# sunbains/scann-rust

Hardware: AMD Instinct MI355X
Metric: QPS @ recall10@10 + achieved HBM GB/s, 1M x 128 f32 (higher is better)
Workload: dtype f32; 1 GPU; AsymmetricHasher LUT16 S=32 K=16 + exact re-rank; n=1000000, n_per_gpu=1000000, dim=128, k=10, batch=1024, global_batch=1024, caller_streams=2, pre_reorder_k=5000, distribution=uniform, parallelism=single GPU

## Files before the change

include/scann_hip.h:

```cpp
#ifndef SCANN_HIP_H
#define SCANN_HIP_H

#include <stddef.h>
#include <stdint.h>

#ifdef __cplusplus
extern "C" {
#endif

typedef enum {
    SCANN_HIP_OK = 0,
    SCANN_HIP_CANCELLED = 1,
    SCANN_HIP_UNKNOWN = 2,
    SCANN_HIP_INVALID_ARGUMENT = 3,
    SCANN_HIP_DEADLINE_EXCEEDED = 4,
    SCANN_HIP_NOT_FOUND = 5,
    SCANN_HIP_ALREADY_EXISTS = 6,
    SCANN_HIP_PERMISSION_DENIED = 7,
    SCANN_HIP_RESOURCE_EXHAUSTED = 8,
    SCANN_HIP_FAILED_PRECONDITION = 9,
    SCANN_HIP_ABORTED = 10,
    SCANN_HIP_OUT_OF_RANGE = 11,
    SCANN_HIP_UNIMPLEMENTED = 12,
    SCANN_HIP_INTERNAL = 13,
// ... 63 lines not shown
    uint32_t pre_reorder_k;
    int32_t exact_reorder;
    uint32_t *tokens;
    float *token_dists;
    uint32_t *cand_idx;
    float *cand_dist;
    uint32_t *cand_count;
    const uint64_t *allow_bitmap;
    uint64_t allow_bitmap_bits;
    int32_t bf_exact;
} scann_hip_search_opts;

void scann_hip_search_opts_default(scann_hip_search_opts *opts);

int scann_hip_search_batched(scann_hip_index *index, const float *queries, uint32_t nq,
                             uint32_t q_stride, uint32_t q_dim, uint32_t k,
                             const scann_hip_search_opts *opts, uint32_t *out_idx,
                             float *out_dist, uint32_t *out_count);

int scann_hip_search_batched_params(scann_hip_index *index, const float *queries, uint32_t nq,
                                    uint32_t q_stride, uint32_t q_dim, const uint32_t *k_per_query,
                                    const scann_hip_search_opts *opts, uint32_t out_pitch,
                                    uint32_t *out_idx, float *out_dist, uint32_t *out_count);

int scann_hip_index_reserve(scann_hip_index *index, uint32_t max_nq, uint32_t max_k,
                            const scann_hip_search_opts *opts);
int scann_hip_search_batched_device(scann_hip_index *index, const float *d_queries,
                                    uint32_t nq, uint32_t q_stride, uint32_t k,
                                    const scann_hip_search_opts *opts, uint32_t *d_out_idx,
                                    float *d_out_dist, uint32_t *d_out_count,
                                    void *hip_stream);
int scann_hip_index_last_device_status(scann_hip_index *index, void *hip_stream);
int scann_hip_index_debug_filter_bounds(scann_hip_index *index, void *hip_stream, uint32_t nq, uint64_t *out_bounds);

#define SCANN_HIP_CROWD_MAX_DEPTH 8192
#define SCANN_HIP_CROWD_MAX_SLOTS 12288
uint32_t scann_hip_crowd_table_slots(uint32_t depth);
int scann_hip_index_set_crowding_attributes(scann_hip_index *index, const uint64_t *attrs, uint64_t n_attrs);
int scann_hip_search_crowded(scann_hip_index *index, const float *queries, uint32_t nq, uint32_t q_stride,
                             uint32_t q_dim, uint32_t k, uint32_t depth, uint32_t per_crowd_limit,
                             const scann_hip_search_opts *opts, uint32_t *out_idx, float *out_dist,
                             uint32_t *out_count);
int scann_hip_index_reserve_crowded(scann_hip_index *index, uint32_t max_nq, uint32_t max_k, uint32_t max_depth,
                                    const scann_hip_search_opts *opts);
int scann_hip_search_crowded_device(scann_hip_index *index, const float *d_queries, uint32_t nq, uint32_t q_stride,
                                    uint32_t k, uint32_t depth, uint32_t per_crowd_limit,
                                    const scann_hip_search_opts *opts, uint32_t *d_out_idx, float *d_out_dist,
                                    uint32_t *d_out_count, void *hip_stream);

#define SCANN_HIP_CROWD_MAX_DIMS 8
int scann_hip_index_set_crowding_attributes_md(scann_hip_index *index, const uint64_t *attrs, uint32_t n_dims,
                                               uint64_t n_attrs);
int scann_hip_search_crowded_md(scann_hip_index *index, const float *queries, uint32_t nq, uint32_t q_stride,
                                uint32_t q_dim, uint32_t k, uint32_t depth, const uint32_t *limits, uint32_t n_limits,
                                const scann_hip_search_opts *opts, uint32_t *out_idx, float *out_dist,
                                uint32_t *out_count);
int scann_hip_search_crowded_md_device(scann_hip_index *index, const float *d_queries, uint32_t nq, uint32_t q_stride,
                                       uint32_t k, uint32_t depth, const uint32_t *limits, uint32_t n_limits,
                                       const scann_hip_search_opts *opts, uint32_t *d_out_idx, float *d_out_dist,
                                       uint32_t *d_out_count, void *hip_stream);
int scann_hip_crowd_md_apply(scann_hip_index *index, const uint32_t *rows_idx, const float *rows_dist,
                             const uint32_t *rows_count, uint32_t nq, uint32_t depth, uint32_t k, const uint32_t *limits,
                             uint32_t n_limits, uint32_t *out_idx, float *out_dist, uint32_t *out_count);

#define SCANN_HIP_MMR_MAX_DEPTH 2048
int scann_hip_search_mmr(scann_hip_index *index, const float *queries, uint32_t nq, uint32_t q_stride, uint32_t q_dim,
// ... 148 lines not shown
```

scann_rust_amd/csrc/api.hip:

```cpp
#include <algorithm>
#include <cmath>
#include <cstddef>
#include <cstdio>
#include <cstdlib>
#include <atomic>
#include <chrono>
#include <cstring>
#include <memory>
#include <mutex>
#include <string>
#include <vector>

#include "bf.h"
#include "comm.h"
#include "common.h"
#include "crowd.h"
#include "index_arrays.h"
#include "mmr.h"
#include "mutable.h"
#include "knobs.h"
#include "launch.h"
#include "txh.h"

namespace scann {
// ... 990 lines not shown
    const uint64_t rtp = (uint64_t)kResThreads * kScanPPT;
    const uint64_t res_chunks_per_leaf = std::max<uint64_t>(1, (t.n_local / std::max(1u, L)) / rtp);
    const uint64_t qgroups = std::max<uint64_t>(1, (quads_per_leaf + kResQuads - 1) / kResQuads);
    const uint64_t units = (t.n_local / rtp + L) * qgroups;
    p.res_cl = (uint32_t)std::min<uint64_t>(64, std::max<uint64_t>(8, units / 4096));
    const bool res_layout = t.code_bits == 4 && t.S <= 32;
    bool resident = res_layout && res_chunks_per_leaf >= 8 && quads_per_leaf >= 32 && units / p.res_cl >= 1536;
    if (kn.resident == 0) resident = false;
    if (kn.resident == 2) resident = res_layout;
    if (kn.res_cl) p.res_cl = kn.res_cl;
    const bool mfma_ok = t.code_bits == 4 && !p.no_threshold && !t.exact_scan;
    const bool sparse = (uint64_t)m * 128 <= stream;
    TxhScan mfma = TxhScan::Gather;
    if (mfma_ok && sparse) mfma = quads_per_leaf >= 6 ? TxhScan::Mfma32 : quads_per_leaf >= 2 ? TxhScan::Mfma16 : TxhScan::Gather;
    if (kn.mfma == 0) mfma = TxhScan::Gather;
    if (kn.mfma == 2) mfma = mfma_ok ? TxhScan::Mfma32 : TxhScan::Gather;
    if (kn.mfma == 3) mfma = mfma_ok ? TxhScan::Mfma16 : TxhScan::Gather;
    if (mfma_ok && t.codes_sp && quads_per_leaf >= 2 && t.n_local / std::max(1u, L) >= 4096 && kn.smfmac &&
        kn.mfma != 0 && kn.mfma != 3)
        mfma = TxhScan::Smfmac;
    if (mfma == TxhScan::Mfma32 && t.codes_sp && kn.smfmac) mfma = TxhScan::Smfmac;
    p.scan = t.exact_scan ? TxhScan::Exact : mfma != TxhScan::Gather ? mfma : resident ? TxhScan::Resident : TxhScan::Gather;
    if (txh_scan_is_mfma(p.scan)) {
        p.cap32 = (uint32_t)std::min<uint64_t>(ms, (uint64_t)p.cap * 4 + 16384);
    }
    p.sp_words = kn.sp_words < 0 ? !t.ah_mode : kn.sp_words != 0;
    p.codes_in_list = t.ah_mode != 0;
    p.thr_ties = kn.thr_ties;
    p.thr_tail = kn.thr_tail && !p.no_threshold && sample_rank(m, p.st) <= kThrTailMaxRank && p.scap > 4096;
    p.sample_mfma = kn.sample_mfma && p.thr_tail && p.thr_ties && txh_scan_is_mfma(p.scan) && t.ah_mode && t.L == 1 &&
                    P == 1 && t.code_bits == 4;
    p.select_direct = kn.select_direct;
    p.use_i8 = t.rows8 && exact_reorder && m >= kn.rerank_i8_min && m > 4 * k;
    p.local_prune = kn.local_prune;
    *out = p;
    return SCANN_HIP_OK;
}

static const char *txh_kernel_name(const TxhIndexDev &t, const TxhPlan &p, bool pinned) {
    if (pinned) return p.pipeline == TxhPipeline::Wide ? "wide_scan_kernel" : "small_scan_kernel";
    switch (p.scan) {
        case TxhScan::Exact: return "leaf_exact_scan_kernel";
        case TxhScan::Mfma16: return "adc_mfma16_kernel";
        case TxhScan::Smfmac: return t.S > 32 ? "adc_smfmac_wide_kernel" : "adc_smfmac_kernel";
        case TxhScan::Mfma32: return "adc_mfma_kernel";
        case TxhScan::Resident: return "adc_scan_res_kernel";
        default: return "adc_scan_kernel";
    }
}

}

int scann::txh_resolve_m(scann_hip_index *ix, uint32_t k, const scann_hip_search_opts *opts, uint32_t *out_m) {
    if (!ix || ix->kind != KIND_TXH) return fail(SCANN_HIP_INVALID_ARGUMENT, "not a tree index");
    scann_hip_search_opts o;
    if (opts) o = *opts; else scann_hip_search_opts_default(&o);
    o.exact_reorder = 1;
    TxhPlan p;
    SCANN_TRY(plan_txh_search(ix, k, &o, 0, false, TxhPipeline::Staged, read_knobs(), &p));
    *out_m = p.m;
    return SCANN_HIP_OK;
}

extern "C" {

static int ensure_txh_workspace(scann_hip_index *ix, TxhWorkspace &s, const TxhPlan &p, bool own_queries,
// ... 634 lines not shown
    for (auto &d : ix->dslots)
        if (d.used && d.key == st && d.ws) {
            ws = d.ws;
            bfw = d.bfw;
        }
    if (ix->kind == KIND_BF) return bf_last_status(*bfw, st);
    if (ix->kind != KIND_TXH || !ws->counters.p) return SCANN_HIP_OK;
    uint32_t counters[CNT_N];
    SCANN_HIP_CHECK(hipMemcpyAsync(counters, ws->counters.p, sizeof(counters),
                                   hipMemcpyDeviceToHost, st));
    SCANN_HIP_CHECK(hipStreamSynchronize(st));
    if (counters[CNT_STATUS] != SCANN_HIP_OK)
        return fail((int)counters[CNT_STATUS],
                    "candidate threshold/buffer miss on the device path (use the host entry "
                    "point, which retries without a threshold and with a full-size buffer)");
    return SCANN_HIP_OK;
}

int scann_hip_index_debug_filter_bounds(scann_hip_index *ix, void *hip_stream, uint32_t nq, uint64_t *out_bounds) {
    if (!ix || ix->kind != KIND_TXH) return fail(SCANN_HIP_INVALID_ARGUMENT, "not a tree / hasher index");
    if (nq && !out_bounds) return fail(SCANN_HIP_INVALID_ARGUMENT, "out_bounds is null");
    SCANN_TRY(set_device(ix->ctx));
    hipStream_t st = static_cast<hipStream_t>(hip_stream);
    std::lock_guard<std::mutex> lock(ix->mu);
    const TxhWorkspace *ws = &ix->ws;
    for (auto &d : ix->dslots)
        if (d.used && d.key == st && d.ws) ws = d.ws;
    if (!ws->thr.p || ws->thr.bytes < (size_t)nq * 8)
        return fail(SCANN_HIP_OUT_OF_RANGE, "no batched search of that many queries has run in this workspace");
    SCANN_HIP_CHECK(hipMemcpy(out_bounds, ws->thr.p, (size_t)nq * 8, hipMemcpyDeviceToHost));
    return SCANN_HIP_OK;
}

uint32_t scann_hip_crowd_table_slots(uint32_t depth) { return crowd_table_slots(depth); }

int scann_hip_index_set_crowding_attributes(scann_hip_index *ix, const uint64_t *attrs, uint64_t n_attrs) {
    if (!ix) return fail(SCANN_HIP_INVALID_ARGUMENT, "index is null");
    if (n_attrs && !attrs) return fail(SCANN_HIP_INVALID_ARGUMENT, "attrs is null");
    std::lock_guard<std::mutex> lock(ix->mu);
    SCANN_TRY(set_device(ix->ctx));
    SCANN_HIP_CHECK(hipDeviceSynchronize());
    ix->crowd_attrs.release();
    ix->n_crowd_attrs = 0;
    ix->has_crowd_attrs = false;
    if (n_attrs == 0) return SCANN_HIP_OK;
    SCANN_TRY(upload(ix->crowd_attrs, attrs, (size_t)n_attrs * 8));
    ix->n_crowd_attrs = n_attrs;
    ix->has_crowd_attrs = true;
    return SCANN_HIP_OK;
}

int scann_hip_index_set_crowding_attributes_md(scann_hip_index *ix, const uint64_t *attrs, uint32_t n_dims,
                                               uint64_t n_attrs) {
    if (!ix) return fail(SCANN_HIP_INVALID_ARGUMENT, "index is null");
    if (n_dims == 0 || n_dims > kCrowdMaxDims)
        return fail(SCANN_HIP_INVALID_ARGUMENT, "crowding dimensions must be 1.." + std::to_string(kCrowdMaxDims));
    if (n_attrs && !attrs) return fail(SCANN_HIP_INVALID_ARGUMENT, "attrs is null");
    std::lock_guard<std::mutex> lock(ix->mu);
    SCANN_TRY(set_device(ix->ctx));
    SCANN_HIP_CHECK(hipDeviceSynchronize());
    ix->crowd_md_attrs.release();
    ix->n_crowd_md_attrs = 0;
    ix->crowd_md_dims = 0;
    if (n_attrs == 0) return SCANN_HIP_OK;
    SCANN_TRY(upload(ix->crowd_md_attrs, attrs, (size_t)n_dims * n_attrs * 8));
    ix->n_crowd_md_attrs = n_attrs;
// ... 695 lines not shown
```

scann_rust_amd/csrc/knobs.h:

```cpp
#pragma once

#include <stdint.h>
#include <stdlib.h>
#include <string.h>

#include <algorithm>

extern char **environ;

namespace scann {

struct Knobs {
    int device_slots = 2;
    uint32_t search_slots = 4;
    const char *rccl_lib = nullptr;
    bool smfmac = true;
    int rerank_i8 = 1;
    bool rerank_fp8 = false;
    int rerank_uniform = 1;
    uint32_t bf_shortlist_min_rows = 65536;
    bool load_pin = true;
    bool small = true;
    int wide = 1;
    int resident = 1;
    uint32_t res_cl = 0;
    int mfma = 1;
    uint32_t rerank_i8_min = 512;
    int sp_words = -1;
    bool thr_ties = true;
    bool thr_tail = true;
    bool sample_mfma = true;
    bool fused = true;
    bool select_direct = true;
    bool local_prune = true;
    double comm_fill = 2.5;
    double bf_shortlist_tail = 1e-6;
    uint32_t bf_shortlist_min_queries = 32;
    int bf_filter = 0;
    double bf_filter_compact_max = 1.0;
};

inline Knobs read_knobs() {
    Knobs k;
    uint32_t seen = 0;
    for (char **ep = environ; ep && *ep; ++ep) {
        const char *e = *ep;
        if (strncmp(e, "SCANN_HIP_", 10) != 0) continue;
        const char *eq = strchr(e, '=');
        if (!eq) continue;
        const size_t n = (size_t)(eq - e);
        const char *v = eq + 1;
        int bit = 0;
        auto is = [&](const char *s) {
            const int b = bit++;
            if (strlen(s) != n || memcmp(s, e, n) != 0 || ((seen >> b) & 1u)) return false;
            seen |= 1u << b;
            return true;
        };
        if (is("SCANN_HIP_DEVICE_SLOTS")) k.device_slots = atoi(v);
        else if (is("SCANN_HIP_SEARCH_SLOTS")) k.search_slots = (uint32_t)std::max(1, std::min(64, atoi(v)));
        else if (is("SCANN_HIP_RCCL_LIB")) k.rccl_lib = v;
        else if (is("SCANN_HIP_SMFMAC")) k.smfmac = atoi(v) != 0;
        else if (is("SCANN_HIP_RERANK_I8")) k.rerank_i8 = atoi(v);
        else if (is("SCANN_HIP_RERANK_STORE")) k.rerank_fp8 = strcmp(v, "fp8") == 0;
        else if (is("SCANN_HIP_RERANK_UNIFORM")) k.rerank_uniform = atoi(v);
        else if (is("SCANN_HIP_BF_SHORTLIST_MIN_ROWS")) k.bf_shortlist_min_rows = (uint32_t)strtoul(v, nullptr, 10);
        else if (is("SCANN_HIP_LOAD_PIN")) k.load_pin = atoi(v) != 0;
        else if (is("SCANN_HIP_SMALL")) k.small = atoi(v) != 0;
        else if (is("SCANN_HIP_WIDE")) k.wide = atoi(v);
        else if (is("SCANN_HIP_RESIDENT")) k.resident = atoi(v);
        else if (is("SCANN_HIP_RES_CL")) k.res_cl = (uint32_t)std::max(1, atoi(v));
        else if (is("SCANN_HIP_MFMA")) k.mfma = atoi(v);
        else if (is("SCANN_HIP_RERANK_I8_MIN")) k.rerank_i8_min = (uint32_t)std::max(1, atoi(v));
        else if (is("SCANN_HIP_SP_WORDS")) k.sp_words = atoi(v) != 0 ? 1 : 0;
        else if (is("SCANN_HIP_THR_TIES")) k.thr_ties = atoi(v) != 0;
        else if (is("SCANN_HIP_THR_TAIL")) k.thr_tail = atoi(v) != 0;
        else if (is("SCANN_HIP_SAMPLE_MFMA")) k.sample_mfma = atoi(v) != 0;
        else if (is("SCANN_HIP_FUSED")) k.fused = atoi(v) != 0;
        else if (is("SCANN_HIP_SELECT_DIRECT")) k.select_direct = atoi(v) != 0;
        else if (is("SCANN_HIP_LOCAL_PRUNE")) k.local_prune = atoi(v) != 0;
        else if (is("SCANN_HIP_COMM_FILL")) {
            const double f = atof(v);
            k.comm_fill = f < 0.0 ? 0.0 : f;
        } else if (is("SCANN_HIP_BF_SHORTLIST_TAIL")) {
            const double t = atof(v);
            if (t > 0.0 && t < 1.0) k.bf_shortlist_tail = t;
        } else if (is("SCANN_HIP_BF_SHORTLIST_MIN_QUERIES")) k.bf_shortlist_min_queries = (uint32_t)strtoul(v, nullptr, 10);
        else if (is("SCANN_HIP_BF_FILTER")) k.bf_filter = atoi(v);
        else if (is("SCANN_HIP_BF_FILTER_COMPACT_MAX")) {
            const double f = atof(v);
            if (f >= 0.0 && f <= 1.0) k.bf_filter_compact_max = f;
        }
    }
    return k;
}

}
```

scann_rust_amd/csrc/txh.h:

```cpp
#pragma once
#include "common.h"

namespace scann {

constexpr uint32_t kScanThreads = 256;
#ifndef SCANN_SCAN_PPT
#define SCANN_SCAN_PPT 2
#endif
constexpr uint32_t kScanPPT = SCANN_SCAN_PPT;
constexpr uint32_t kScanTP = kScanThreads * kScanPPT;
constexpr uint32_t kScanQuadsPerTile = 32;
#ifndef SCANN_SCAN_DEPTH
#define SCANN_SCAN_DEPTH 1
#endif
#ifndef SCANN_SCAN_WAVES
#define SCANN_SCAN_WAVES 6
#endif
constexpr uint32_t kScanDepth = SCANN_SCAN_DEPTH;
constexpr uint32_t kScanWaves = SCANN_SCAN_WAVES;
constexpr uint32_t kResThreads = 512;
constexpr uint32_t kResQuads = 4;
constexpr uint32_t kSortCap = 16384;
#ifndef SCANN_SAMPLE_TARGET
#define SCANN_SAMPLE_TARGET 32768
// ... 84 lines not shown

enum {
    CNT_TOTAL_QUADS = 0, CNT_TOTAL_TILES = 1, CNT_QUEUE_HEAD = 2, CNT_STATUS = 3,
    CNT_TOTAL_STILES = 4, CNT_SQUEUE_HEAD = 5, CNT_N = 8,
    CNT_XQ = 32, CNT_XQ_STRIDE = 32, CNT_XS = CNT_XQ + 8 * CNT_XQ_STRIDE ,
    CNT_WORDS = CNT_XS + 8 * CNT_XQ_STRIDE
};

enum class TxhPipeline : uint8_t { Staged, Small, Wide };
enum class TxhScan : uint8_t { Gather, Resident, Mfma32, Mfma16, Smfmac, Exact };

struct TxhPlan {
    uint32_t nq, P, m, k;
    uint32_t cap;
    bool exact_reorder;
    bool no_threshold;
    TxhPipeline pipeline;
    TxhScan scan;
    uint32_t st, scap, sqpt;
    uint32_t qpt;
    uint32_t res_cl;
    uint32_t cap32;
    bool sp_words;
    bool codes_in_list;
    bool thr_ties;
    bool thr_tail;
    bool sample_mfma;
    bool fused;
    uint32_t chunk, grid;
    uint32_t small_max_leaf;
    uint32_t wide_cap2;
    bool select_direct;
    bool use_i8;
    bool local_prune;
};

struct TxhWork : TxhPlan {
    uint32_t q_stride;
    int need_sorted_cands;
    const uint64_t *allow;
    uint64_t allow_bits;
    const float *queries;
    float *cdist;
    uint32_t *tokens;
    float *token_dists;
    uint32_t *vbase;
    uint32_t *rr_lb, *rr_ub;
    int8_t *lut8;
    void *lut8_meta;
    int *mfma_thr1;
    uint32_t *cand32_cnt;
    uint32_t *cand32;
    uint32_t *cand32_codes;
    uint32_t *small_done;
    uint32_t small_seq;
    uint32_t *small_tickets;
    uint32_t *wide_min;
    uint64_t *wide_ckey;
    uint32_t *wide_ceb;
    uint32_t *wide_cidx;
    uint32_t *wide_cnt;
    uint32_t *sbase;
    uint32_t *pair_sbase;
    uint32_t *stile_off;
    uint32_t *samp;
    uint32_t *leaf_cnt;
// ... 76 lines not shown
```

scann_rust_amd/csrc/txh_rows.hip:

```cpp
#include "launch.h"
#include "txh_stages.h"

namespace scann {

__global__ __launch_bounds__(256) void rows_i8_build_kernel(const float *__restrict__ rows, uint64_t n, uint32_t dim,
                                                            uint32_t stride, int8_t *__restrict__ rows8,
                                                            float2 *__restrict__ meta, float uni_scale) {
    const uint64_t r = (uint64_t)blockIdx.x * 32 + (threadIdx.x >> 3);
    const uint32_t l8 = threadIdx.x & 7u;
    const bool act = r < n;
    const float *row = rows + (act ? r : 0) * stride;
    float mx = 0.0f;
    for (uint32_t j = l8; j < dim; j += 8) mx = fmaxf(mx, fabsf(row[j]));
    mx = fmaxf(mx, __shfl_xor(mx, 1, 8));
    mx = fmaxf(mx, __shfl_xor(mx, 2, 8));
    mx = fmaxf(mx, __shfl_xor(mx, 4, 8));
    const bool finite = mx < __builtin_inff();
    const float sc = uni_scale > 0.0f ? uni_scale : (mx > 0.0f && finite) ? mx / 127.0f : 1.0f;
    float err = 0.0f;
    for (uint32_t j = l8; j < dim; j += 8) {
        const float x = row[j];
        float t = rintf(x / sc);
        t = fminf(fmaxf(t, -127.0f), 127.0f);
        if (act) rows8[r * dim + j] = (int8_t)(t == t ? (int)t : 0);
// ... 89 lines not shown
    uint32_t bad = 0;
    for (uint32_t j = l8; j < dim; j += 8) {
        const float x = row[j];
        const uint32_t b = fp8_from_f32(x * scale, 0);
        const float hw = __builtin_amdgcn_cvt_f32_fp8((int)b, 0);
        bad += (__float_as_uint(hw) != __float_as_uint(fp8_to_f32(b, 0))) ? 1u : 0u;
        if (act) rows8[r * dim + j] = (uint8_t)b;
        const float e = x - hw * inv;
        err = err + e * e;
    }
    err += __shfl_xor(err, 1, 8);
    err += __shfl_xor(err, 2, 8);
    err += __shfl_xor(err, 4, 8);
    if (act && bad) atomicAdd(mismatch, bad);
    if (act && l8 == 0) {
        float E = sqrtf(err) * 1.0001f + 1e-30f;
        if (!(E == E) || !finite) E = __builtin_inff();
        meta[r] = make_float2(inv, E);
    }
}

struct I8RerankArgs {
    const int8_t *rows8;
    const float2 *meta;
    float uni_scale, uni_E;
    const float *queries;
    uint32_t q_stride, m;
    const uint32_t *cand_row, *cand_count;
    uint32_t *lb, *ub;
};

constexpr uint32_t kI8PerBlock = 256;

template <int FMT, bool UNI = false>
__global__ __launch_bounds__(256) void rerank_i8_kernel(uint32_t dim, I8RerankArgs a) {
    typedef float v2f __attribute__((ext_vector_type(2)));
    extern __shared__ __attribute__((aligned(16))) float s_q[];
    const uint32_t q = blockIdx.y, tid = threadIdx.x;
    const uint32_t nsel = a.cand_count[q];
    const uint32_t c0 = blockIdx.x * kI8PerBlock;
    if (c0 >= nsel) return;
    for (uint32_t j = tid; j < dim; j += 256) s_q[j] = a.queries[(size_t)q * a.q_stride + j];
    __syncthreads();
    const uint32_t l8 = tid & 7u;
    constexpr int R = kI8PerBlock / 32;
    uint32_t row[R];
#pragma unroll
    for (int it = 0; it < R; ++it) {
        const uint32_t c = c0 + (uint32_t)it * 32u + (tid >> 3);
        row[it] = c < nsel ? a.cand_row[(size_t)q * a.m + c] : 0u;
    }
#pragma unroll
    for (int it = 0; it < R; ++it) {
        const uint32_t c = c0 + (uint32_t)it * 32u + (tid >> 3);
        const bool act = c < nsel;
        const float2 me = UNI ? make_float2(a.uni_scale, a.uni_E) : a.meta[row[it]];
        const int8_t *r8 = a.rows8 + (size_t)row[it] * dim;
        float acc = 0.0f;
        for (uint32_t j0 = l8 * 16u; j0 < dim; j0 += 128u) {
            const uint4 v = *reinterpret_cast<const uint4 *>(r8 + j0);
            const uint32_t w[4] = {v.x, v.y, v.z, v.w};
            if constexpr (FMT == 1) {
#pragma unroll
                for (int wi = 0; wi < 4; ++wi) {
                    const v2f lo = __builtin_amdgcn_cvt_pk_f32_fp8((int)w[wi], false);
                    const v2f hi = __builtin_amdgcn_cvt_pk_f32_fp8((int)w[wi], true);
                    const float xs[4] = {lo.x, lo.y, hi.x, hi.y};
#pragma unroll
                    for (int i = 0; i < 4; ++i) {
                        const float d = s_q[j0 + wi * 4 + i] - xs[i] * me.x;
                        acc = fmaf(d, d, acc);
                    }
                }
            } else {
#pragma unroll
                for (int i = 0; i < 16; ++i) {
                    const float x = me.x * (float)(int)(int8_t)(w[i >> 2] >> (8 * (i & 3)));
                    const float d = s_q[j0 + i] - x;
                    acc = fmaf(d, d, acc);
                }
            }
        }
        acc += __shfl_xor(acc, 1, 8);
        acc += __shfl_xor(acc, 2, 8);
        acc += __shfl_xor(acc, 4, 8);
        if (act && l8 == 0) {
            const float E = me.y;
            const float slack = (2.0f * sqrtf(acc) * E + E * E) * 1.0001f + acc * ((float)(dim + 8) * 1.2e-7f) + 1e-30f;
            float L = acc - slack, U = acc + slack;
            if (!(slack < __builtin_inff()) || !(acc < __builtin_inff())) {
                L = -__builtin_inff();
                U = __builtin_inff();
            }
            a.lb[(size_t)q * a.m + c] = f32_to_ordered(L);
            a.ub[(size_t)q * a.m + c] = f32_to_ordered(U);
        }
    }
}

int launch_rerank_i8(const TxhIndexDev &ix, const TxhWork &w, hipStream_t st) {
    const size_t lds_rr = (size_t)ix.dim * 4;
    I8RerankArgs ia;
    ia.rows8 = ix.rows8; ia.meta = reinterpret_cast<const float2 *>(ix.rows8_meta); ia.queries = w.queries;
    ia.q_stride = w.q_stride; ia.m = w.m; ia.cand_row = w.cand_row; ia.cand_count = w.cand_count;
    ia.lb = w.rr_lb; ia.ub = w.rr_ub;
    ia.uni_scale = ix.rows8_scale; ia.uni_E = ix.rows8_emax;
    return with_value<1, 2, 0>(ix.rows8_fmt == 1 ? 1 : ix.rows8_uniform ? 2 : 0, [&](auto v) {
        return launch((rerank_i8_kernel<v() == 1 ? 1 : 0, v() == 2>), dim3(ceil_div_u32(w.m, kI8PerBlock), w.nq),
                      dim3(256), lds_rr, st, ix.dim, ia);
    });
}

int launch_rows_fp8_build(const float *d_rows, uint64_t n, uint32_t dim, uint32_t stride, uint8_t *d_rows8,
                          void *d_meta, uint32_t *d_mismatch, hipStream_t st) {
    if (n == 0) return SCANN_HIP_OK;
    SCANN_TRY(launch(rows_fp8_build_kernel, dim3((uint32_t)ceil_div_u64(n, 32)), dim3(256), 0, st, d_rows, n, dim,
                     stride, d_rows8, reinterpret_cast<float2 *>(d_meta), d_mismatch));
    return SCANN_HIP_OK;
}

int launch_fp8_quantize(const float *d_values, uint64_t n, float scale, int format, uint8_t *d_out, hipStream_t st) {
    if (n == 0) return SCANN_HIP_OK;
    SCANN_TRY(launch(fp8_quantize_kernel, dim3((uint32_t)std::min<uint64_t>(ceil_div_u64(n, 256), 65535)), dim3(256), 0,
                     st, d_values, n, scale, format, d_out));
    return SCANN_HIP_OK;
}

int launch_fp8_dequantize(const uint8_t *d_bits, uint64_t n, float scale, int format, float *d_out, hipStream_t st) {
    if (n == 0) return SCANN_HIP_OK;
    SCANN_TRY(launch(fp8_dequantize_kernel, dim3((uint32_t)std::min<uint64_t>(ceil_div_u64(n, 256), 65535)), dim3(256),
                     0, st, d_bits, n, scale, format, d_out));
    return SCANN_HIP_OK;
}

int launch_fp8_one_to_many(const float *d_query, uint32_t dim, const uint8_t *d_db, uint64_t stride, uint64_t n,
                           int dot, float *d_out, hipStream_t st) {
    if (n == 0) return SCANN_HIP_OK;
    const size_t lds = (size_t)dim * sizeof(float);
    SCANN_TRY(launch(fp8_one_to_many_kernel, dim3((uint32_t)std::min<uint64_t>(ceil_div_u64(n, 256), 65535)),
                     dim3(256), lds, st, d_query, dim, d_db, stride, n, dot, d_out));
    return SCANN_HIP_OK;
}
// ... 11 lines not shown
```

scann_rust_amd/hip.py:

```python
import ctypes as C
import os

import numpy as np

_HERE = os.path.dirname(os.path.abspath(__file__))
LIB_PATH = os.environ.get("SCANN_HIP_LIB") or os.path.join(_HERE, "libscann_hip.so")

OK, INVALID_ARGUMENT, RESOURCE_EXHAUSTED, FAILED_PRECONDITION = 0, 3, 8, 9
NOT_FOUND, ABORTED = 5, 10
OUT_OF_RANGE, UNIMPLEMENTED, INTERNAL, UNAVAILABLE = 11, 12, 13, 14
SQUARED_L2, L2, DOT_PRODUCT, L1, COSINE = 0, 1, 2, 3, 4
MMR_MAX_DEPTH = 2048
CROWD_MAX_DIMS = 8
MUTABLE_MAX_CAPACITY = 65536
MUTABLE_MAX_K = 2048
MUTABLE_DELTA_TILE = 1024
FOLD_CHUNK = 1024

_CODE_NAMES = {
    0: "Ok", 1: "Cancelled", 2: "Unknown", 3: "InvalidArgument", 4: "DeadlineExceeded",
    5: "NotFound", 6: "AlreadyExists", 7: "PermissionDenied", 8: "ResourceExhausted",
    9: "FailedPrecondition", 10: "Aborted", 11: "OutOfRange", 12: "Unimplemented",
    13: "Internal", 14: "Unavailable", 15: "DataLoss", 16: "Unauthenticated",
}

EXPORTS = [
    "scann_hip_init", "scann_hip_shutdown", "scann_hip_last_error", "scann_hip_version",
    "scann_hip_compute_stride", "scann_hip_bf_create", "scann_hip_bf_create_quantized", "scann_hip_bf16_quantize",
    "scann_hip_txh_create",
    "scann_hip_search_opts_default", "scann_hip_search_batched", "scann_hip_search_batched_params", "scann_hip_index_reserve",
    "scann_hip_search_batched_device", "scann_hip_index_last_device_status", "scann_hip_index_debug_filter_bounds",
    "scann_hip_crowd_table_slots", "scann_hip_index_set_crowding_attributes", "scann_hip_search_crowded",
    "scann_hip_index_reserve_crowded", "scann_hip_search_crowded_device",
    "scann_hip_index_set_crowding_attributes_md", "scann_hip_search_crowded_md", "scann_hip_search_crowded_md_device",
    "scann_hip_crowd_md_apply",
    "scann_hip_search_mmr", "scann_hip_search_mmr_device", "scann_hip_index_reserve_mmr", "scann_hip_mmr_apply",
    "scann_hip_txh_search_local_device", "scann_hip_txh_merge_device",
    "scann_hip_assign_leaves", "scann_hip_txh_partition", "scann_hip_lut_from_query",
    "scann_hip_adc_distances", "scann_hip_lut16_distances_batch", "scann_hip_encode",
    "scann_hip_fp8_quantize", "scann_hip_fp8_dequantize", "scann_hip_fp8_distances",
    "scann_hip_bf_distances", "scann_hip_bf_search_radius", "scann_hip_bf_search_radius_opts", "scann_hip_allow_bitmap_count", "scann_hip_bf_assign_nearest",
    "scann_hip_kmeans_init_pp", "scann_hip_kmeans_lloyd", "scann_hip_txh_pack_blocks_device", "scann_hip_index_size", "scann_hip_index_dimensionality",
    "scann_hip_index_destroy", "scann_hip_index_enable_timing",
    "scann_hip_index_last_kernel_ms",
    "scann_hip_txh_write_file", "scann_hip_bf_write_file", "scann_hip_index_file_info",
    "scann_hip_index_load_file",
    "scann_hip_abi_layout", "scann_hip_lut16_quantize",
    "scann_hip_comm_unique_id", "scann_hip_comm_create", "scann_hip_comm_destroy",
    "scann_hip_txh_search_sharded_device", "scann_hip_comm_last_status", "scann_hip_comm_layout",
    "scann_hip_mutable_create", "scann_hip_mutable_destroy", "scann_hip_mutable_add", "scann_hip_mutable_remove",
    "scann_hip_mutable_update", "scann_hip_mutable_get", "scann_hip_mutable_exists", "scann_hip_mutable_size",
    "scann_hip_mutable_pending", "scann_hip_mutable_needs_rebuild", "scann_hip_mutable_search",
    "scann_hip_mutable_export_live", "scann_hip_mutable_rebase", "scann_hip_mutable_enable_timing",
    "scann_hip_mutable_last_stage_ms", "scann_hip_fold_mutable", "scann_hip_fold_mutable_stage_ms",
    "scann_hip_index_write_file",
]


class ScannError(RuntimeError):

    def __init__(self, code, message):
        super().__init__("%s: %s" % (_CODE_NAMES.get(code, str(code)), message))
        self.code = code
        self.message = message
# ... 54 lines not shown
        return _lib
    if not os.path.exists(LIB_PATH):
        raise ScannError(UNAVAILABLE, "libscann_hip.so is not built (run "
                         "`python -m scann_rust_amd.build`); there is no CPU fallback")
    L = C.CDLL(LIB_PATH)
    L.scann_hip_init.argtypes = [C.c_int, C.POINTER(vp)]
    L.scann_hip_shutdown.argtypes = [vp]
    L.scann_hip_shutdown.restype = None
    L.scann_hip_last_error.restype = C.c_char_p
    L.scann_hip_version.restype = C.c_char_p
    L.scann_hip_compute_stride.restype = C.c_uint32
    L.scann_hip_compute_stride.argtypes = [C.c_uint32]
    L.scann_hip_bf_create.argtypes = [vp, f32p, C.c_uint64, C.c_uint32, C.c_uint32, C.c_int,
                                      C.POINTER(vp)]
    L.scann_hip_bf_create_quantized.argtypes = [vp, vp, C.c_uint64, C.c_uint32, C.c_uint32, C.c_int, C.c_float,
                                                C.c_int, C.POINTER(vp)]
    L.scann_hip_bf16_quantize.argtypes = [vp, f32p, C.c_uint64, u16p]
    L.scann_hip_txh_create.argtypes = [vp, C.POINTER(TxhDesc), C.POINTER(vp)]
    L.scann_hip_txh_write_file.argtypes = [C.c_char_p, C.POINTER(TxhDesc)]
    L.scann_hip_bf_write_file.argtypes = [C.c_char_p, f32p, C.c_uint64, C.c_uint32, C.c_uint32, C.c_int]
    L.scann_hip_index_file_info.argtypes = [C.c_char_p, C.POINTER(FileInfo)]
    L.scann_hip_index_load_file.argtypes = [vp, C.c_char_p, C.POINTER(vp)]
    L.scann_hip_search_opts_default.argtypes = [C.POINTER(SearchOpts)]
    L.scann_hip_search_opts_default.restype = None
    L.scann_hip_search_batched.argtypes = [vp, f32p, C.c_uint32, C.c_uint32, C.c_uint32,
                                           C.c_uint32, C.POINTER(SearchOpts), u32p, f32p, u32p]
    L.scann_hip_search_batched_params.argtypes = [vp, f32p, C.c_uint32, C.c_uint32, C.c_uint32, u32p,
                                                  C.POINTER(SearchOpts), C.c_uint32, u32p, f32p, u32p]
    L.scann_hip_index_reserve.argtypes = [vp, C.c_uint32, C.c_uint32, C.POINTER(SearchOpts)]
    L.scann_hip_search_batched_device.argtypes = [vp, vp, C.c_uint32, C.c_uint32, C.c_uint32,
                                                  C.POINTER(SearchOpts), vp, vp, vp, vp]
    L.scann_hip_index_last_device_status.argtypes = [vp, vp]
    L.scann_hip_index_debug_filter_bounds.argtypes = [vp, vp, C.c_uint32, u64p]
    L.scann_hip_crowd_table_slots.restype = C.c_uint32
    L.scann_hip_crowd_table_slots.argtypes = [C.c_uint32]
    L.scann_hip_index_set_crowding_attributes.argtypes = [vp, u64p, C.c_uint64]
    L.scann_hip_search_crowded.argtypes = [vp, f32p, C.c_uint32, C.c_uint32, C.c_uint32, C.c_uint32, C.c_uint32,
                                           C.c_uint32, C.POINTER(SearchOpts), u32p, f32p, u32p]
    L.scann_hip_index_reserve_crowded.argtypes = [vp, C.c_uint32, C.c_uint32, C.c_uint32, C.POINTER(SearchOpts)]
    L.scann_hip_search_crowded_device.argtypes = [vp, vp, C.c_uint32, C.c_uint32, C.c_uint32, C.c_uint32, C.c_uint32,
                                                  C.POINTER(SearchOpts), vp, vp, vp, vp]
    L.scann_hip_index_set_crowding_attributes_md.argtypes = [vp, u64p, C.c_uint32, C.c_uint64]
    L.scann_hip_search_crowded_md.argtypes = [vp, f32p, C.c_uint32, C.c_uint32, C.c_uint32, C.c_uint32, C.c_uint32,
                                              u32p, C.c_uint32, C.POINTER(SearchOpts), u32p, f32p, u32p]
    L.scann_hip_search_crowded_md_device.argtypes = [vp, vp, C.c_uint32, C.c_uint32, C.c_uint32, C.c_uint32, u32p,
                                                     C.c_uint32, C.POINTER(SearchOpts), vp, vp, vp, vp]
    L.scann_hip_crowd_md_apply.argtypes = [vp, u32p, f32p, u32p, C.c_uint32, C.c_uint32, C.c_uint32, u32p, C.c_uint32,
                                           u32p, f32p, u32p]
    L.scann_hip_search_mmr.argtypes = [vp, f32p, C.c_uint32, C.c_uint32, C.c_uint32, C.c_uint32, C.c_uint32, C.c_float,
                                       C.POINTER(SearchOpts), u32p, f32p, u32p]
    L.scann_hip_search_mmr_device.argtypes = [vp, vp, C.c_uint32, C.c_uint32, C.c_uint32, C.c_uint32, C.c_float,
                                              C.POINTER(SearchOpts), vp, vp, vp, vp]
    L.scann_hip_index_reserve_mmr.argtypes = [vp, C.c_uint32, C.c_uint32, C.c_uint32, C.POINTER(SearchOpts)]
    L.scann_hip_mmr_apply.argtypes = [vp, u32p, f32p, u32p, C.c_uint32, C.c_uint32, C.c_uint32, C.c_float,
                                      u32p, f32p, u32p]
    L.scann_hip_txh_search_local_device.argtypes = [vp, vp, C.c_uint32, C.c_uint32, C.c_uint32,
                                                    C.POINTER(SearchOpts), vp, vp, vp, vp, vp]
    L.scann_hip_txh_merge_device.argtypes = [vp, C.c_uint32, C.c_uint32, C.c_uint32, C.c_uint32,
                                             C.c_uint32, C.c_uint64, vp, vp, vp, vp, vp, vp, vp, vp, vp]
    L.scann_hip_assign_leaves.argtypes = [u32p, C.c_uint32, C.c_uint32, u32p]
    L.scann_hip_txh_partition.argtypes = [vp, f32p, C.c_uint32, C.c_uint32, C.c_uint32,
                                          C.c_uint32, u32p, f32p, u32p]
    L.scann_hip_lut_from_query.argtypes = [vp, f32p, C.c_uint32, C.c_uint32, u32p, f32p]
    L.scann_hip_adc_distances.argtypes = [vp, f32p, C.c_uint32, f32p]
    L.scann_hip_lut16_distances_batch.argtypes = [vp, u8p, u8p, C.c_uint32, C.c_uint64,
                                                  C.c_float, C.c_float, f32p]
# ... 285 lines not shown

    def search_mmr_device(self, d_queries, nq, q_stride, k, depth, lam, d_out_idx, d_out_dist, d_out_count, stream,
                          opts=None):
        check(load().scann_hip_search_mmr_device(
            self.h, vp(d_queries), nq, q_stride, k, depth, C.c_float(lam), C.byref(opts) if opts is not None else None,
            vp(d_out_idx), vp(d_out_dist), vp(d_out_count), vp(stream)))

    def reserve_mmr(self, max_nq, max_k, max_depth=0, opts=None):
        check(load().scann_hip_index_reserve_mmr(self.h, max_nq, max_k, max_depth,
                                                 C.byref(opts) if opts is not None else None))

    def mmr_apply(self, rows_idx, rows_dist, rows_count, k, lam):
        return self._staged_apply(
            lambda ri, rd, rc, nq, depth, oi, od, oc: load().scann_hip_mmr_apply(
                self.h, ri, rd, rc, nq, depth, k, C.c_float(lam), oi, od, oc),
            rows_idx, rows_dist, rows_count, k)

    def search_radius(self, query, radius, capacity=None, allow=None, allow_bits=None):
        return bf_search_radius(self, query, radius, capacity, allow=allow, allow_bits=allow_bits)

    def enable_timing(self, on=True):
        load().scann_hip_index_enable_timing(self.h, 1 if on else 0)

    def last_kernel_ms(self):
        name = C.c_char_p()
        ms = load().scann_hip_index_last_kernel_ms(self.h, C.byref(name))
        return float(ms), (name.value or b"").decode()

    def debug_filter_bounds(self, nq, stream=0):
        out = np.zeros(nq, np.uint64)
        check(load().scann_hip_index_debug_filter_bounds(self.h, vp(stream), nq, ptr(out, u64p)))
        return out


class Mutable:

    def __init__(self, base, capacity, device=0):
        h = vp()
        check(load().scann_hip_mutable_create(context(device), base.h, int(capacity), C.byref(h)))
        self.h = h
        self.base = base
        self.dim = base.dimensionality()
        self.stride = compute_stride(self.dim)

    def close(self):
        if self.h:
            load().scann_hip_mutable_destroy(self.h)
            self.h = None

    def __del__(self):
        try:
            self.close()
        except Exception:
            pass

    @staticmethod
    def _rows(rows):
        r = f32(rows)
        return r[None] if r.ndim == 1 else r

    def add(self, rows):
        r = self._rows(rows)
        ids = np.zeros(r.shape[0], np.uint32)
        check(load().scann_hip_mutable_add(self.h, ptr(r, f32p), r.shape[0], r.shape[1], r.shape[1], ptr(ids, u32p)))
        return int(ids[0]) if np.ndim(rows) == 1 else ids

# ... 430 lines not shown
```

Baseline: 1.497 million queries/s.

## Expand int8 re-rank distance algebraically and transpose lane reductions with DPP

```diff
diff --git a/include/scann_hip.h b/include/scann_hip.h
--- a/include/scann_hip.h
+++ b/include/scann_hip.h
@@ -119,6 +119,8 @@
                                     void *hip_stream);
 int scann_hip_index_last_device_status(scann_hip_index *index, void *hip_stream);
 int scann_hip_index_debug_filter_bounds(scann_hip_index *index, void *hip_stream, uint32_t nq, uint64_t *out_bounds);
+int scann_hip_index_debug_rerank_brackets(scann_hip_index *index, void *hip_stream, uint32_t nq, uint32_t m, uint32_t *out_lb,
+                                          uint32_t *out_ub, uint32_t *out_rows, uint32_t *out_counts);
 
 #define SCANN_HIP_CROWD_MAX_DEPTH 8192
 #define SCANN_HIP_CROWD_MAX_SLOTS 12288
diff --git a/scann_rust_amd/csrc/api.hip b/scann_rust_amd/csrc/api.hip
--- a/scann_rust_amd/csrc/api.hip
+++ b/scann_rust_amd/csrc/api.hip
@@ -1046,6 +1046,7 @@
                     P == 1 && t.code_bits == 4;
     p.select_direct = kn.select_direct;
     p.use_i8 = t.rows8 && exact_reorder && m >= kn.rerank_i8_min && m > 4 * k;
+    p.i8_expand = kn.rerank_expand;
     p.local_prune = kn.local_prune;
     *out = p;
     return SCANN_HIP_OK;
@@ -1746,6 +1747,28 @@
     return SCANN_HIP_OK;
 }
 
+int scann_hip_index_debug_rerank_brackets(scann_hip_index *ix, void *hip_stream, uint32_t nq, uint32_t m, uint32_t *out_lb,
+                                          uint32_t *out_ub, uint32_t *out_rows, uint32_t *out_counts) {
+    if (!ix || ix->kind != KIND_TXH) return fail(SCANN_HIP_INVALID_ARGUMENT, "not a tree / hasher index");
+    if (nq && m && (!out_lb || !out_ub || !out_rows || !out_counts))
+        return fail(SCANN_HIP_INVALID_ARGUMENT, "an output is null");
+    SCANN_TRY(set_device(ix->ctx));
+    hipStream_t st = static_cast<hipStream_t>(hip_stream);
+    std::lock_guard<std::mutex> lock(ix->mu);
+    const TxhWorkspace *ws = &ix->ws;
+    for (auto &d : ix->dslots)
+        if (d.used && d.key == st && d.ws) ws = d.ws;
+    const size_t list = (size_t)nq * m * 4;
+    if (!ws->rr_lb.p || !ws->rr_ub.p || !ws->cand_row.p || !ws->cand_count.p || ws->rr_lb.bytes < list ||
+        ws->rr_ub.bytes < list || ws->cand_row.bytes < list || ws->cand_count.bytes < (size_t)nq * 4)
+        return fail(SCANN_HIP_OUT_OF_RANGE, "no filtered re-rank of that many queries and candidates has run in this workspace");
+    SCANN_HIP_CHECK(hipMemcpy(out_lb, ws->rr_lb.p, list, hipMemcpyDeviceToHost));
+    SCANN_HIP_CHECK(hipMemcpy(out_ub, ws->rr_ub.p, list, hipMemcpyDeviceToHost));
+    SCANN_HIP_CHECK(hipMemcpy(out_rows, ws->cand_row.p, list, hipMemcpyDeviceToHost));
+    SCANN_HIP_CHECK(hipMemcpy(out_counts, ws->cand_count.p, (size_t)nq * 4, hipMemcpyDeviceToHost));
+    return SCANN_HIP_OK;
+}
+
 uint32_t scann_hip_crowd_table_slots(uint32_t depth) { return crowd_table_slots(depth); }
 
 int scann_hip_index_set_crowding_attributes(scann_hip_index *ix, const uint64_t *attrs, uint64_t n_attrs) {
diff --git a/scann_rust_amd/csrc/knobs.h b/scann_rust_amd/csrc/knobs.h
--- a/scann_rust_amd/csrc/knobs.h
+++ b/scann_rust_amd/csrc/knobs.h
@@ -26,6 +26,7 @@
     uint32_t res_cl = 0;
     int mfma = 1;
     uint32_t rerank_i8_min = 512;
+    bool rerank_expand = true;
     int sp_words = -1;
     bool thr_ties = true;
     bool thr_tail = true;
@@ -72,6 +73,7 @@
         else if (is("SCANN_HIP_RES_CL")) k.res_cl = (uint32_t)std::max(1, atoi(v));
         else if (is("SCANN_HIP_MFMA")) k.mfma = atoi(v);
         else if (is("SCANN_HIP_RERANK_I8_MIN")) k.rerank_i8_min = (uint32_t)std::max(1, atoi(v));
+        else if (is("SCANN_HIP_RERANK_EXPAND")) k.rerank_expand = atoi(v) != 0;
         else if (is("SCANN_HIP_SP_WORDS")) k.sp_words = atoi(v) != 0 ? 1 : 0;
         else if (is("SCANN_HIP_THR_TIES")) k.thr_ties = atoi(v) != 0;
         else if (is("SCANN_HIP_THR_TAIL")) k.thr_tail = atoi(v) != 0;
diff --git a/scann_rust_amd/csrc/txh.h b/scann_rust_amd/csrc/txh.h
--- a/scann_rust_amd/csrc/txh.h
+++ b/scann_rust_amd/csrc/txh.h
@@ -140,6 +140,7 @@
     uint32_t wide_cap2;
     bool select_direct;
     bool use_i8;
+    bool i8_expand;
     bool local_prune;
 };
 
diff --git a/scann_rust_amd/csrc/txh_rows.hip b/scann_rust_amd/csrc/txh_rows.hip
--- a/scann_rust_amd/csrc/txh_rows.hip
+++ b/scann_rust_amd/csrc/txh_rows.hip
@@ -145,7 +145,43 @@
 
 constexpr uint32_t kI8PerBlock = 256;
 
-template <int FMT, bool UNI = false>
+constexpr int kDppXor1 = 0xB1, kDppXor2 = 0x4E, kDppHalfMirror = 0x141;
+template <int CTRL> __device__ __forceinline__ int dpp_get(int v) { return __builtin_amdgcn_update_dpp(0, v, CTRL, 0xF, 0xF, true); }
+template <int CTRL> __device__ __forceinline__ float dpp_get(float v) {
+    return __int_as_float(__builtin_amdgcn_update_dpp(0, __float_as_int(v), CTRL, 0xF, 0xF, true));
+}
+
+__device__ __forceinline__ float sum8(float v) {
+    v += dpp_get<kDppXor1>(v);
+    v += dpp_get<kDppXor2>(v);
+    return v + dpp_get<kDppHalfMirror>(v);
+}
+
+template <typename T> __device__ __forceinline__ T sum8_transposed(const T (&v)[8], uint32_t l8) {
+    const bool h4 = l8 & 4u, h2 = l8 & 2u, h1 = l8 & 1u;
+    T a[4], b[2];
+#pragma unroll
+    for (int i = 0; i < 4; ++i) a[i] = (h4 ? v[i + 4] : v[i]) + dpp_get<kDppHalfMirror>(h4 ? v[i] : v[i + 4]);
+#pragma unroll
+    for (int i = 0; i < 2; ++i) b[i] = (h2 ? a[i + 2] : a[i]) + dpp_get<kDppXor2>(h2 ? a[i] : a[i + 2]);
+    return (h1 ? b[1] : b[0]) + dpp_get<kDppXor1>(h1 ? b[0] : b[1]);
+}
+
+template <bool EXPANDED>
+__device__ __forceinline__ void store_bracket(const I8RerankArgs &a, size_t at, uint32_t dim, float acc, float E, float B) {
+    const float slack = EXPANDED ? (2.0f * sqrtf(fmaxf(acc, 0.0f) + B) * E + E * E) * 1.0001f +
+                                       fabsf(acc) * ((float)(dim + 8) * 1.2e-7f) + B + 1e-30f
+                                 : (2.0f * sqrtf(acc) * E + E * E) * 1.0001f + acc * ((float)(dim + 8) * 1.2e-7f) + 1e-30f;
+    float L = acc - slack, U = acc + slack;
+    if (!(slack < __builtin_inff()) || !(acc < __builtin_inff())) {
+        L = -__builtin_inff();
+        U = __builtin_inff();
+    }
+    a.lb[at] = f32_to_ordered(L);
+    a.ub[at] = f32_to_ordered(U);
+}
+
+template <int FMT, bool UNI = false, int EX = 0>
 __global__ __launch_bounds__(256) void rerank_i8_kernel(uint32_t dim, I8RerankArgs a) {
     typedef float v2f __attribute__((ext_vector_type(2)));
     extern __shared__ __attribute__((aligned(16))) float s_q[];
@@ -163,50 +199,129 @@
         const uint32_t c = c0 + (uint32_t)it * 32u + (tid >> 3);
         row[it] = c < nsel ? a.cand_row[(size_t)q * a.m + c] : 0u;
     }
-#pragma unroll
-    for (int it = 0; it < R; ++it) {
-        const uint32_t c = c0 + (uint32_t)it * 32u + (tid >> 3);
-        const bool act = c < nsel;
-        const float2 me = UNI ? make_float2(a.uni_scale, a.uni_E) : a.meta[row[it]];
-        const int8_t *r8 = a.rows8 + (size_t)row[it] * dim;
-        float acc = 0.0f;
-        for (uint32_t j0 = l8 * 16u; j0 < dim; j0 += 128u) {
-            const uint4 v = *reinterpret_cast<const uint4 *>(r8 + j0);
-            const uint32_t w[4] = {v.x, v.y, v.z, v.w};
-            if constexpr (FMT == 1) {
-#pragma unroll
-                for (int wi = 0; wi < 4; ++wi) {
-                    const v2f lo = __builtin_amdgcn_cvt_pk_f32_fp8((int)w[wi], false);
-                    const v2f hi = __builtin_amdgcn_cvt_pk_f32_fp8((int)w[wi], true);
-                    const float xs[4] = {lo.x, lo.y, hi.x, hi.y};
-#pragma unroll
-                    for (int i = 0; i < 4; ++i) {
-                        const float d = s_q[j0 + wi * 4 + i] - xs[i] * me.x;
+    if constexpr (EX == 0) {
+#pragma unroll
+        for (int it = 0; it < R; ++it) {
+            const uint32_t c = c0 + (uint32_t)it * 32u + (tid >> 3);
+            const bool act = c < nsel;
+            const float2 me = UNI ? make_float2(a.uni_scale, a.uni_E) : a.meta[row[it]];
+            const int8_t *r8 = a.rows8 + (size_t)row[it] * dim;
+            float acc = 0.0f;
+            for (uint32_t j0 = l8 * 16u; j0 < dim; j0 += 128u) {
+                const uint4 v = *reinterpret_cast<const uint4 *>(r8 + j0);
+                const uint32_t w[4] = {v.x, v.y, v.z, v.w};
+                if constexpr (FMT == 1) {
+#pragma unroll
+                    for (int wi = 0; wi < 4; ++wi) {
+                        const v2f lo = __builtin_amdgcn_cvt_pk_f32_fp8((int)w[wi], false);
+                        const v2f hi = __builtin_amdgcn_cvt_pk_f32_fp8((int)w[wi], true);
+                        const float xs[4] = {lo.x, lo.y, hi.x, hi.y};
+#pragma unroll
+                        for (int i = 0; i < 4; ++i) {
+                            const float d = s_q[j0 + wi * 4 + i] - xs[i] * me.x;
+                            acc = fmaf(d, d, acc);
+                        }
+                    }
+                } else {
+#pragma unroll
+                    for (int i = 0; i < 16; ++i) {
+                        const float x = me.x * (float)(int)(int8_t)(w[i >> 2] >> (8 * (i & 3)));
+                        const float d = s_q[j0 + i] - x;
                         acc = fmaf(d, d, acc);
+                    }
+                }
+            }
+            acc += __shfl_xor(acc, 1, 8);
+            acc += __shfl_xor(acc, 2, 8);
+            acc += __shfl_xor(acc, 4, 8);
+            if (act && l8 == 0) store_bracket<false>(a, (size_t)q * a.m + c, dim, acc, me.y, 0.0f);
+        }
+    } else {
+        const uint32_t ce = c0 + l8 * 32u + (tid >> 3);
+        const bool acte = ce < nsel;
+        const float2 mee = UNI ? make_float2(a.uni_scale, a.uni_E) : a.meta[acte ? a.cand_row[(size_t)q * a.m + ce] : 0u];
+        if constexpr (FMT == 1) {
+            float accv[R];
+#pragma unroll
+            for (int it = 0; it < R; ++it) {
+                const float inv = a.meta[row[it]].x;
+                const int8_t *r8 = a.rows8 + (size_t)row[it] * dim;
+                float acc = 0.0f;
+                for (uint32_t j0 = l8 * 16u; j0 < dim; j0 += 128u) {
+                    const uint4 v = *reinterpret_cast<const uint4 *>(r8 + j0);
+                    const uint32_t w[4] = {v.x, v.y, v.z, v.w};
+#pragma unroll
+                    for (int wi = 0; wi < 4; ++wi) {
+                        const v2f lo = __builtin_amdgcn_cvt_pk_f32_fp8((int)w[wi], false);
+                        const v2f hi = __builtin_amdgcn_cvt_pk_f32_fp8((int)w[wi], true);
+                        const float xs[4] = {lo.x, lo.y, hi.x, hi.y};
+#pragma unroll
+                        for (int i = 0; i < 4; ++i) {
+                            const float d = s_q[j0 + wi * 4 + i] - xs[i] * inv;
+                            acc = fmaf(d, d, acc);
+                        }
+                    }
+                }
+                accv[it] = acc;
+            }
+            const float acc = sum8_transposed(accv, l8);
+            if (acte) store_bracket<false>(a, (size_t)q * a.m + ce, dim, acc, mee.y, 0.0f);
+        } else {
+            constexpr int NP = EX - 1;
+            float qr[NP > 0 ? NP : 1][16];
+            float q2 = 0.0f;
+            if constexpr (NP > 0) {
+#pragma unroll
+                for (int p = 0; p < NP; ++p) {
+                    const uint32_t j0 = l8 * 16u + (uint32_t)p * 128u;
+#pragma unroll
+                    for (int i = 0; i < 16; ++i) {
+                        qr[p][i] = j0 < dim ? s_q[j0 + i] : 0.0f;
+                        q2 = fmaf(qr[p][i], qr[p][i], q2);
                     }
                 }
             } else {
-#pragma unroll
-                for (int i = 0; i < 16; ++i) {
-                    const float x = me.x * (float)(int)(int8_t)(w[i >> 2] >> (8 * (i & 3)));
-                    const float d = s_q[j0 + i] - x;
-                    acc = fmaf(d, d, acc);
+                for (uint32_t j0 = l8 * 16u; j0 < dim; j0 += 128u)
+#pragma unroll
+                    for (int i = 0; i < 16; ++i) q2 = fmaf(s_q[j0 + i], s_q[j0 + i], q2);
+            }
+            q2 = sum8(q2);
+            float Dv[R];
+            int Nv[R];
+#pragma unroll
+            for (int it = 0; it < R; ++it) {
+                const int8_t *r8 = a.rows8 + (size_t)row[it] * dim;
+                float D = 0.0f;
+                int N = 0;
+                auto pass = [&](uint32_t j0, int &Np, auto qat) {
+                    const uint4 v = *reinterpret_cast<const uint4 *>(r8 + j0);
+                    const uint32_t w[4] = {v.x, v.y, v.z, v.w};
+#pragma unroll
+                    for (int wi = 0; wi < 4; ++wi) Np = __builtin_amdgcn_sdot4((int)w[wi], (int)w[wi], Np, false);
+#pragma unroll
+                    for (int i = 0; i < 16; ++i) D = fmaf(qat(i), (float)(int)(int8_t)(w[i >> 2] >> (8 * (i & 3))), D);
+                };
+                if constexpr (NP > 0) {
+#pragma unroll
+                    for (int p = 0; p < NP; ++p) {
+                        const uint32_t j0 = l8 * 16u + (uint32_t)p * 128u;
+                        int Np = 0;
+                        pass(j0 < dim ? j0 : 0u, Np, [&](int i) { return qr[p][i]; });
+                        N += j0 < dim ? Np : 0;
+                    }
+                } else {
+                    for (uint32_t j0 = l8 * 16u; j0 < dim; j0 += 128u) pass(j0, N, [&](int i) { return s_q[j0 + i]; });
                 }
-            }
-        }
-        acc += __shfl_xor(acc, 1, 8);
-        acc += __shfl_xor(acc, 2, 8);
-        acc += __shfl_xor(acc, 4, 8);
-        if (act && l8 == 0) {
-            const float E = me.y;
-            const float slack = (2.0f * sqrtf(acc) * E + E * E) * 1.0001f + acc * ((float)(dim + 8) * 1.2e-7f) + 1e-30f;
-            float L = acc - slack, U = acc + slack;
-            if (!(slack < __builtin_inff()) || !(acc < __builtin_inff())) {
-                L = -__builtin_inff();
-                U = __builtin_inff();
-            }
-            a.lb[(size_t)q * a.m + c] = f32_to_ordered(L);
-            a.ub[(size_t)q * a.m + c] = f32_to_ordered(U);
+                Dv[it] = D;
+                Nv[it] = N;
+            }
+            const float D = sum8_transposed(Dv, l8);
+            const float Nf = (float)sum8_transposed(Nv, l8);
+            const float s = mee.x;
+            const float acc = (q2 - (2.0f * s) * D) + (s * s) * Nf;
+            const float rt = sqrtf(q2) + s * sqrtf(Nf);
+            const float B = rt * rt * ((float)(dim + 8) * 1.2e-7f);
+            if (acte) store_bracket<true>(a, (size_t)q * a.m + ce, dim, acc, mee.y, B);
         }
     }
 }
@@ -218,9 +333,14 @@
     ia.q_stride = w.q_stride; ia.m = w.m; ia.cand_row = w.cand_row; ia.cand_count = w.cand_count;
     ia.lb = w.rr_lb; ia.ub = w.rr_ub;
     ia.uni_scale = ix.rows8_scale; ia.uni_E = ix.rows8_emax;
-    return with_value<1, 2, 0>(ix.rows8_fmt == 1 ? 1 : ix.rows8_uniform ? 2 : 0, [&](auto v) {
-        return launch((rerank_i8_kernel<v() == 1 ? 1 : 0, v() == 2>), dim3(ceil_div_u32(w.m, kI8PerBlock), w.nq),
-                      dim3(256), lds_rr, st, ix.dim, ia);
+    const bool fp8 = ix.rows8_fmt == 1;
+    const int ex = !w.i8_expand || (!fp8 && !ix.rows8_uniform) ? 0 : fp8 || ix.dim > 256 ? 1 : ix.dim <= 128 ? 2 : 3;
+    return with_value<1, 2, 0>(fp8 ? 1 : ix.rows8_uniform ? 2 : 0, [&](auto v) {
+        return with_value<0, 1, 2, 3>(ex, [&](auto e) {
+            constexpr int EX = v() == 0 ? 0 : (v() == 1 && e() > 1) ? 1 : e();
+            return launch((rerank_i8_kernel<v() == 1 ? 1 : 0, v() == 2, EX>), dim3(ceil_div_u32(w.m, kI8PerBlock), w.nq),
+                          dim3(256), lds_rr, st, ix.dim, ia);
+        });
     });
 }
 
diff --git a/scann_rust_amd/hip.py b/scann_rust_amd/hip.py
--- a/scann_rust_amd/hip.py
+++ b/scann_rust_amd/hip.py
@@ -30,6 +30,7 @@
     "scann_hip_txh_create",
     "scann_hip_search_opts_default", "scann_hip_search_batched", "scann_hip_search_batched_params", "scann_hip_index_reserve",
     "scann_hip_search_batched_device", "scann_hip_index_last_device_status", "scann_hip_index_debug_filter_bounds",
+    "scann_hip_index_debug_rerank_brackets",
     "scann_hip_crowd_table_slots", "scann_hip_index_set_crowding_attributes", "scann_hip_search_crowded",
     "scann_hip_index_reserve_crowded", "scann_hip_search_crowded_device",
     "scann_hip_index_set_crowding_attributes_md", "scann_hip_search_crowded_md", "scann_hip_search_crowded_md_device",
@@ -150,6 +151,7 @@
                                                   C.POINTER(SearchOpts), vp, vp, vp, vp]
     L.scann_hip_index_last_device_status.argtypes = [vp, vp]
     L.scann_hip_index_debug_filter_bounds.argtypes = [vp, vp, C.c_uint32, u64p]
+    L.scann_hip_index_debug_rerank_brackets.argtypes = [vp, vp, C.c_uint32, C.c_uint32, u32p, u32p, u32p, u32p]
     L.scann_hip_crowd_table_slots.restype = C.c_uint32
     L.scann_hip_crowd_table_slots.argtypes = [C.c_uint32]
     L.scann_hip_index_set_crowding_attributes.argtypes = [vp, u64p, C.c_uint64]
@@ -501,6 +503,13 @@
         check(load().scann_hip_index_debug_filter_bounds(self.h, vp(stream), nq, ptr(out, u64p)))
         return out
 
+    def debug_rerank_brackets(self, nq, m, stream=0):
+        lb, ub, rows = (np.zeros((nq, m), np.uint32) for _ in range(3))
+        counts = np.zeros(nq, np.uint32)
+        check(load().scann_hip_index_debug_rerank_brackets(self.h, vp(stream), nq, m, ptr(lb, u32p), ptr(ub, u32p),
+                                                           ptr(rows, u32p), ptr(counts, u32p)))
+        return lb, ub, rows, counts
+
 
 class Mutable:
 
```

Result: faster. 1.526 million queries/s (median of 6 runs) (+1.9%).
